# evanwang1990/FMwR

Measured on AMD Instinct MI355X. Metric: training examples/sec, 10Mx1M sparse FM SGD, higher is better.
Workload: dtype f32

## Files before the change

fmwr_amd/csrc/fm_batch_kernels.hip:

```cpp
#include <atomic>
#include <mutex>
#include <utility>
#include <vector>

#include "fmx_internal.h"
#include "fm_probit.h"
#include "fmx_test_hooks.h"

#ifndef FMX_U
#define FMX_U 4
#endif
#ifndef FMX_SPARSE_WAVES
#define FMX_SPARSE_WAVES 4
#endif
#ifndef FMX_DENSE_WAVES
#define FMX_DENSE_WAVES 4
#endif
#ifndef FMX_U_LARGE
#define FMX_U_LARGE 4
#endif
#ifndef FMX_U_SMALL
#define FMX_U_SMALL 8
#endif

// ... 451 lines not shown
#pragma unroll
    for (int i = 0; i < VEC; ++i) pair += 0.5 * (sm[s][i] * sm[s][i] - qm[s][i]);
#pragma unroll
    for (int off = LPR / 2; off > 0; off >>= 1) pair += __shfl_xor(pair, off);
    const double y_hat = lin[s] + pair;
    if constexpr (TRAIN) {
      double mult = 0.0;
      if (have) {
        mult = grad_mult(h, y_hat, a.y[a.r0 + row]);
        float4 srow = slice_make(sm[s], T());
        srow = embed_store<LPR>(srow, lig, (float)mult, a.embed);
        *reinterpret_cast<float4*>(reinterpret_cast<T*>(a.S) + (size_t)row * KP + lig * VEC) = srow;
        if (lig == 0) reinterpret_cast<T*>(a.amul)[row] = (T)mult;
      }
      if (lig == 0) red[s * NG + eg] = mult;
    } else {
      if (have && lig == 0 && a.yhat) a.yhat[row] = link_apply(h, y_hat, a.link, a.pn_y);
    }
  }
  if constexpr (TRAIN) {
    __syncthreads();
    if (tid % 64 == 0) {
      const int s = tid / 64;
      if (R0 + (int64_t)s * NG < a.nrows) {
        double g0 = 0.0, q0 = 0.0;
        for (int i = 0; i < NG; ++i) { const double m = red[s * NG + i]; g0 += m; q0 += m * m; }
        a.partials[2 * ((size_t)blockIdx.x * MERGE_SLOTS + s)] = g0;
        a.partials[2 * ((size_t)blockIdx.x * MERGE_SLOTS + s) + 1] = q0;
      }
    }
  }
}

template <bool UNIFORM, bool PIPE>
__global__ __launch_bounds__(WG_THREADS, 4) void fm_rows_sched_k(RowsArgs a, Hyper h) {
  using T = float;
  constexpr int LPR = 4, VEC = 4, KP = LPR * VEC;
  constexpr int NG = WG_THREADS / LPR;
  constexpr int PER = MERGE_STAGE / WG_THREADS;
  static_assert(MERGE_STAGE == SCHED_STAGE_STEPS * NG && MERGE_SLOTS == 4, "the stage holds SCHED_STAGE_STEPS steps of one word per lane group");
  static_assert(UNIFORM || !PIPE, "only the unrolled walk has a round to request together");
  __shared__ uint32_t stage[MERGE_STAGE];
  __shared__ double red[MERGE_RPW];

  const int tid = threadIdx.x;
  const int gid = tid / LPR;
  const int lig = tid % LPR;
  const int64_t R0 = (int64_t)blockIdx.x * MERGE_RPW;
  const uint32_t w_lo = a.sched_dir[blockIdx.x], w_hi = a.sched_dir[blockIdx.x + 1];
  const int cnt = (w_hi - w_lo < (uint32_t)MERGE_STAGE) ? (int)(w_hi - w_lo) : MERGE_STAGE;
  const int steps = UNIFORM ? (cnt / NG) & ~3 : cnt / NG;
  {
    uint32_t id[PER];
#pragma unroll
    for (int u = 0; u < PER; ++u) {
      const int i = tid + u * WG_THREADS;
      id[u] = i < cnt ? a.sched[(size_t)w_lo + i] : SCHED_BUBBLE;
    }
#pragma unroll
    for (int u = 0; u < PER; ++u) {
      const int i = tid + u * WG_THREADS;
      if (i < cnt) stage[i] = id[u];
    }
  }
  __syncthreads();

  const __amdgpu_buffer_rsrc_t v_rsrc = table_rsrc(a.V, a.sched_vbytes);
  const __amdgpu_buffer_rsrc_t w_rsrc = table_rsrc(a.w ? a.w : a.V, a.w ? a.sched_wbytes : a.sched_vbytes);
  const bool k1 = h.k1 != 0;
  const int vsh = RowStride<T, LPR>::v(a.vsh) + 2, wsh = RowStride<T, LPR>::w(a.wsh) + 2;
  const uint32_t lane_off = (uint32_t)(lig * VEC * sizeof(T));
  double sm[MERGE_SLOTS][VEC], qm[MERGE_SLOTS][VEC], lin[MERGE_SLOTS];
#pragma unroll
  for (int s = 0; s < MERGE_SLOTS; ++s) {
#pragma unroll
    for (int i = 0; i < VEC; ++i) { sm[s][i] = 0.0; qm[s][i] = 0.0; }
    lin[s] = h.k0 ? a.scal[SC_W0] : 0.0;
  }
  const uint32_t* __restrict__ mine = stage + gid;

  if constexpr (UNIFORM) {
    for (int t = 0; t < steps; t += MERGE_SLOTS) {
// ... 28 lines not shown
        for (int i = 0; i < VEC; ++i) { tmp[i] = tmp[i] * x; tsq[i] = tmp[i] * tmp[i]; }
        if (k1) lin[j] += wx;
#pragma unroll
        for (int i = 0; i < VEC; ++i) { sm[j][i] += tmp[i]; qm[j][i] += tsq[i]; }
      }
    }
  } else {
    for (int t = 0; t < steps; ++t) {
      const uint32_t wd = mine[t * NG];
      const bool live = wd != SCHED_BUBBLE;
      const uint32_t c = wd & SCHED_MAX_P;
      const int esl = live ? (int)(wd >> 30) : MERGE_SLOTS;
      const float4 vv = buf_row(v_rsrc, live ? (c << vsh) + lane_off : BUF_SKIP, T());
      const T wv = buf_elem(w_rsrc, live ? c << wsh : BUF_SKIP, T());
      const double x = 1.0;
      const double wx = (double)wv * x;
      double tmp[VEC], tsq[VEC];
      slice_get(vv, tmp);
#pragma unroll
      for (int i = 0; i < VEC; ++i) { tmp[i] = tmp[i] * x; tsq[i] = tmp[i] * tmp[i]; }
#pragma unroll
      for (int s = 0; s < MERGE_SLOTS; ++s) {
        if (esl == s) {
          if (k1) lin[s] += wx;
#pragma unroll
          for (int i = 0; i < VEC; ++i) { sm[s][i] += tmp[i]; qm[s][i] += tsq[i]; }
        }
      }
    }
  }

  int eg = tid / LPR;
  asm volatile("" : "+v"(eg));
#pragma unroll
  for (int s = 0; s < MERGE_SLOTS; ++s) {
    const int64_t row = R0 + s * NG + eg;
    const bool have = row < a.nrows;
    double pair = 0.0;
#pragma unroll
    for (int i = 0; i < VEC; ++i) pair += 0.5 * (sm[s][i] * sm[s][i] - qm[s][i]);
#pragma unroll
    for (int off = LPR / 2; off > 0; off >>= 1) pair += __shfl_xor(pair, off);
    const double y_hat = lin[s] + pair;
    double mult = 0.0;
    if (have) {
      mult = grad_mult(h, y_hat, a.y[a.r0 + row]);
      float4 srow = slice_make(sm[s], T());
      srow = embed_store<LPR>(srow, lig, (float)mult, a.embed);
      *reinterpret_cast<float4*>(reinterpret_cast<T*>(a.S) + (size_t)row * KP + lig * VEC) = srow;
      if (lig == 0) reinterpret_cast<T*>(a.amul)[row] = (T)mult;
    }
    if (lig == 0) red[s * NG + eg] = mult;
  }
  __syncthreads();
  if (tid % 64 == 0) {
    const int s = tid / 64;
    if (R0 + (int64_t)s * NG < a.nrows) {
      double g0 = 0.0, q0 = 0.0;
      for (int i = 0; i < NG; ++i) { const double m = red[s * NG + i]; g0 += m; q0 += m * m; }
      a.partials[2 * ((size_t)blockIdx.x * MERGE_SLOTS + s)] = g0;
      a.partials[2 * ((size_t)blockIdx.x * MERGE_SLOTS + s) + 1] = q0;
    }
  }
}

template <typename T, int LPR, bool TRAIN>
__global__ __launch_bounds__(WG_THREADS) void fm_rows_forward_dyn_k(RowsArgs a, Hyper h) {
  using vec_t = typename Slice<T>::vec;
  constexpr int VEC = Slice<T>::N;
  constexpr int KP = LPR * VEC;
  constexpr int GROUPS = WG_THREADS / LPR;
  constexpr int RPW = 4 * GROUPS;
  constexpr int RU = FMX_U_LARGE;
  constexpr int PER = (RU + LPR - 1) / LPR;
  __shared__ int next_row;
  __shared__ double red[TRAIN ? RPW : 1];
  const int tid = threadIdx.x;
  const int grp = tid / LPR, lig = tid % LPR;
  const int lane0 = (tid & 63) - lig;
  const int64_t R0 = (int64_t)blockIdx.x * RPW;
  const int rows_here = (int)((R0 + RPW < a.nrows ? R0 + RPW : a.nrows) - R0);
  if (tid == 0) next_row = GROUPS;
  if (TRAIN) for (int i = tid; i < RPW; i += WG_THREADS) red[i] = 0.0;
  __syncthreads();
  const T* __restrict__ Vt = reinterpret_cast<const T*>(a.V) + lig * VEC;
// ... 433 lines not shown
template <bool TRAIN, int U>
static int launch_rows_merged_u(fmx_engine* e, const RowsArgs& a, int mode, bool* ran) {
  const size_t v_bytes = ((size_t)e->p << a.vsh) * sizeof(float);
  if (mode != 2 && (a.nrows < rows_merged_fill<TRAIN, U>(e) || a.col_skew != 1 || v_bytes <= MERGE_MIN_TABLE)) return FMX_OK;
  bool fits = false;
  FMX_TRY(rows_merged_fits(e, a, &fits));
  if (!fits) { g_rows_merged[1]++; return FMX_OK; }
  const int64_t grid = (a.nrows + MERGE_RPW - 1) / MERGE_RPW;
  FMX_CHECK(grid < (1LL << 31), FMX_ERR_INVALID, "rows_forward: grid too large (%lld)", (long long)grid);
  hipLaunchKernelGGL((fm_rows_merged_k<float, 4, TRAIN, U>), dim3((unsigned)grid), dim3(WG_THREADS), 0, e->stream, a, e->hyper);
  FMX_HIP(hipGetLastError());
  g_rows_merged[0]++;
  *ran = true;
  return FMX_OK;
}

template <bool TRAIN>
static int launch_rows_merged(fmx_engine* e, const RowsArgs& a, bool fp64_tables, bool* ran) {
  *ran = false;
  const int mode = rows_merge_mode();
  if (mode == 0 || fp64_tables || e->kp32 != 16 || !a.unit || a.qout || a.no_w || a.wg_threads == 64 || a.sort_rows || a.flat == 1) return FMX_OK;
  if (TRAIN && e->cfg.task == FMX_TASK_RANKING) return FMX_OK;
  if (a.nrows <= 0 || a.max_row_len <= 0 || a.mat_uid == 0) return FMX_OK;
  switch (rows_merge_u()) {
    case 2: return launch_rows_merged_u<TRAIN, 2>(e, a, mode, ran);
    default: return launch_rows_merged_u<TRAIN, 1>(e, a, mode, ran);
  }
}

#ifndef FMX_ROWS_SCHED_DEFAULT
#define FMX_ROWS_SCHED_DEFAULT 1
#endif
#ifndef FMX_ROWS_SCHED_POLICY_DEFAULT
#define FMX_ROWS_SCHED_POLICY_DEFAULT SCHED_MERGE
#endif
#ifndef FMX_ROWS_SCHED_RHO_DEFAULT
#define FMX_ROWS_SCHED_RHO_DEFAULT 1024
#endif
static std::atomic<int64_t> g_rows_sched[3];
void debug_rows_sched_launches(int64_t out[3]) {
  for (int i = 0; i < 3; ++i) out[i] = g_rows_sched[i].load();
}
void rows_sched_count_build() { g_rows_sched[2]++; }
static int rows_sched_mode() {
  static const int v = [] { const char* s = getenv("FMX_ROWS_SCHED"); return s ? atoi(s) : (getenv("FMX_ROWS_MERGE") ? 0 : FMX_ROWS_SCHED_DEFAULT); }();
  return v;
}
static int rows_sched_policy() {
  static const int v = [] {
    const char* s = getenv("FMX_ROWS_SCHED_POLICY");
    if (!s) return (int)FMX_ROWS_SCHED_POLICY_DEFAULT;
    return s[0] == 'm' ? (int)SCHED_MERGE : s[0] == 'f' ? (int)SCHED_FRONT : s[0] == 'r' ? (int)SCHED_ROUND : (int)FMX_ROWS_SCHED_POLICY_DEFAULT;
  }();
  return v;
}
static int rows_sched_rho_q() {
  static const int v = [] {
    const char* s = getenv("FMX_ROWS_SCHED_RHO");
    if (!s) return (int)FMX_ROWS_SCHED_RHO_DEFAULT;
    const double r = atof(s);
    return r <= 0.0 ? 0 : r >= 1.0 ? 1024 : (int)(r * 1024.0 + 0.5);
  }();
  return v;
}
static int rows_sched_u() { static const int v = [] { const char* s = getenv("FMX_ROWS_SCHED_U"); return (s && atoi(s) == 4) ? 4 : 1; }(); return v; }

bool rows_sched_wanted(fmx_engine* e, const RowsArgs& a, int* policy, int* rho_q) {
  const int mode = rows_sched_mode();
  if (mode == 0 || mb_wide(e) || e->kp32 != 16 || !a.unit || a.qout || a.no_w || a.wg_threads == 64 || a.sort_rows || a.flat == 1) return false;
  if (e->cfg.task == FMX_TASK_RANKING || a.nrows <= 0 || a.max_row_len <= 0 || a.mat_uid == 0 || !a.w) return false;
  const uint64_t v_bytes = (uint64_t)e->p * (uint64_t)a.vs * sizeof(float), w_bytes = (uint64_t)e->p * (uint64_t)a.ws * sizeof(float);
  if (v_bytes >= BUF_SKIP || w_bytes >= BUF_SKIP || e->p > SCHED_MAX_P) return false;
  if (mode != 2 && (a.nrows < rows_merged_fill<true, 1>(e) || a.col_skew != 1 || v_bytes <= MERGE_MIN_TABLE)) return false;
  *policy = rows_sched_policy();
  *rho_q = *policy == SCHED_MERGE ? 0 : rows_sched_rho_q();
  return true;
}

static int launch_rows_sched(fmx_engine* e, const RowsArgs& a_in, bool* ran) {
  *ran = false;
  if (a_in.sched_state == 0) return FMX_OK;
  int policy = 0, rho_q = 0;
  if (!rows_sched_wanted(e, a_in, &policy, &rho_q)) return FMX_OK;
  if (a_in.sched_state != 1 || !a_in.sched || !a_in.sched_dir) { g_rows_sched[1]++; return FMX_OK; }
  RowsArgs a = a_in;
  a.sched_vbytes = (uint32_t)((uint64_t)e->p * (uint64_t)a.vs * sizeof(float));
  a.sched_wbytes = (uint32_t)((((uint64_t)e->p - 1) * (uint64_t)a.ws + 1) * sizeof(float));
  const int64_t grid = (a.nrows + MERGE_RPW - 1) / MERGE_RPW;
  FMX_CHECK(grid < (1LL << 31), FMX_ERR_INVALID, "rows_forward: grid too large (%lld)", (long long)grid);
  if (!a.sched_uniform) hipLaunchKernelGGL((fm_rows_sched_k<false, false>), dim3((unsigned)grid), dim3(WG_THREADS), 0, e->stream, a, e->hyper);
  else if (rows_sched_u() == 4) hipLaunchKernelGGL((fm_rows_sched_k<true, true>), dim3((unsigned)grid), dim3(WG_THREADS), 0, e->stream, a, e->hyper);
  else hipLaunchKernelGGL((fm_rows_sched_k<true, false>), dim3((unsigned)grid), dim3(WG_THREADS), 0, e->stream, a, e->hyper);
  FMX_HIP(hipGetLastError());
  g_rows_sched[0]++;
  *ran = true;
  return FMX_OK;
}

int launch_rows_forward(fmx_engine* e, const RowsArgs& a_in, bool train, bool fp64_tables) {
  RowsArgs a = a_in;
  FMX_CHECK(a.vs >= (fp64_tables ? e->kp64 : e->kp32) && a.ws >= 1 && (a.vs & (a.vs - 1)) == 0 && (a.ws & (a.ws - 1)) == 0, FMX_ERR_STATE,
            "rows_forward: table strides not set (%d, %d)", a.vs, a.ws);
  {
    const int kp = fp64_tables ? e->kp64 : e->kp32;
    FMX_CHECK((!fp64_tables && kp <= WIR_MAX_KP) || (a.vs == kp && a.ws == 1), FMX_ERR_STATE, "rows_forward: strides (%d, %d) on a table of compiled strides (%d, 1)",
              a.vs, a.ws, kp);
  }
  a.vsh = __builtin_ctz((unsigned)a.vs); a.wsh = __builtin_ctz((unsigned)a.ws);
  static const bool embed_ok = [] { const char* v = getenv("FMX_EMBED_MULT"); return !(v && v[0] == '0'); }();
  static const int force = [] { const char* v = getenv("FMX_ROWS_SERIAL"); return v ? atoi(v) : -1; }();
  RowsTune& tu = e->rows_tune;
  auto pick = [&](const RowsArgs& r, int* serial, int* trial) -> int {
    *trial = -1;
    *serial = 1;
    if (force >= 0) { *serial = force; return FMX_OK; }
    const bool timed = r.wg_threads != 64 && r.nrows >= RowsTune::MIN_ROWS;
    const int64_t key = r.unit ? 1 : 0;
    if (timed && key != tu.key) {
      if (tu.events && tu.launches > 0 && tu.decided < 0) FMX_HIP(hipStreamSynchronize(e->stream));
      tu.key = key; tu.decided = -1; tu.launches = 0;
    }
    if (tu.decided >= 0) { *serial = tu.decided; return FMX_OK; }
    if (!timed) return FMX_OK;
// ... 1271 lines not shown
```

fmwr_amd/csrc/fm_ingest.hip:

```cpp
#include <hip/hip_runtime.h>

#include <atomic>
#include <mutex>
#include <thread>
#include <type_traits>
#include <vector>
#include <cstring>

#include <rocprim/rocprim.hpp>

#include "fmx_internal.h"

namespace fmx {

static std::atomic<int> g_fail_next_plan_build{0};
void debug_fail_next_plan_build() { g_fail_next_plan_build.store(1); }

__device__ __forceinline__ uint32_t entry_row(const int64_t* __restrict__ row_ptr, int64_t r0, int64_t nrows, int64_t base, int64_t t, int fixed_len) {
  if (fixed_len > 0) return (uint32_t)((t - base) / fixed_len);
  int64_t lo = r0, hi = r0 + nrows;
  while (hi - lo > 1) {
    const int64_t mid = (lo + hi) >> 1;
    if (row_ptr[mid] <= t) lo = mid; else hi = mid;
  }
// ... 1057 lines not shown
  FMX_HIP(hipHostMalloc(&L.h_counts, (size_t)(nt > 0 ? nt : 1) * 4 * sizeof(uint32_t)));
  PlanWorkspace ws;
  FMX_TRY(ws.reserve(max_cnt, m->p, stream));
  L.plans.resize((size_t)nt);
  for (int64_t t = 0; t < nt; ++t) {
    fmx_matrix::TilePlan& pl = L.plans[(size_t)t];
    const int64_t base = h_ptr[(size_t)t], cnt = h_ptr[(size_t)t + 1] - base;
    FMX_TRY(plan_alloc(pl, m->p, cnt, cnt >= (int64_t)m->p));
    pl.r0 = tile_start[(size_t)t]; pl.nrows = tile_start[(size_t)t + 1] - pl.r0; pl.base = base; pl.cnt = cnt;
    FMX_TRY(plan_build(pl, ws, m->p, m->row_ptr, m->col, m->val, L.brow, L.bval, stream, m->unit_values, m->fixed_row_len, m->dense_prefix,
                       m->field_base.empty() ? nullptr : &m->field_base));
    FMX_HIP(hipMemcpyAsync(L.h_counts + 4 * t, pl.dcounts, 4 * sizeof(uint32_t), hipMemcpyDeviceToHost, stream));
  }
  FMX_HIP(hipStreamSynchronize(stream));
  int64_t max_seg = 0;
  for (int64_t t = 0; t < nt; ++t) {
    plan_set_counts(L.plans[(size_t)t], m->p, L.h_counts + 4 * t);
    if ((int64_t)L.plans[(size_t)t].n_seg > max_seg) max_seg = L.plans[(size_t)t].n_seg;
  }
  m->plans.swap(L.plans);
  m->brow = L.brow; L.brow = nullptr;
  m->bval = L.bval; L.bval = nullptr;
  m->step_first_tile.swap(step_first);
  m->batch_rows = batch_rows; m->tile_rows = tile_rows; m->n_batches = nb;
  m->max_long_seg = max_seg; m->max_tile_cnt = max_cnt;
  m->plan_generation++;
  return FMX_OK;
}

constexpr int SCHED_IDS = 9216;
static std::atomic<uint32_t> g_sched_id_limit{SCHED_MAX_P};
void debug_rows_sched_id_limit(uint32_t limit) { g_sched_id_limit.store(limit ? limit : SCHED_MAX_P); }

template <bool WRITE>
__global__ __launch_bounds__(WG_THREADS) void rows_sched_k(const int64_t* __restrict__ row_ptr, const uint32_t* __restrict__ col, int64_t r0, int64_t nrows, uint32_t p,
                                                           int policy, uint32_t rho_q, uint32_t* __restrict__ steps, const uint32_t* __restrict__ dir,
                                                           uint32_t* __restrict__ words) {
  constexpr int NG = 64, SLOTS = 4, RPW = NG * SLOTS;
  __shared__ uint32_t ids[SCHED_IDS];
  __shared__ uint32_t most[NG];
  const int tid = threadIdx.x;
  const int64_t R0 = (int64_t)blockIdx.x * RPW;
  const int64_t R1 = R0 + RPW < nrows ? R0 + RPW : nrows;
  const int64_t lo = row_ptr[r0 + R0], hi = row_ptr[r0 + R1];
  const bool fits_lds = hi - lo <= SCHED_IDS;
  const int cnt = fits_lds ? (int)(hi - lo) : 0;
  for (int i = tid; i < cnt; i += WG_THREADS) ids[i] = col[lo + i];
  int pos[SLOTS], end[SLOTS], left = 0;
  if (tid < NG) {
#pragma unroll
    for (int s = 0; s < SLOTS; ++s) {
      const int64_t row = R0 + s * NG + tid;
      const int64_t ra = row < nrows ? row : nrows, rb = row + 1 < nrows ? row + 1 : nrows;
      const int64_t ta = row_ptr[r0 + ra] - lo, tb = row_ptr[r0 + rb] - lo;
      pos[s] = (int)(ta < cnt ? ta : cnt);
      end[s] = (int)(tb < cnt ? tb : cnt);
      left += end[s] - pos[s];
    }
    most[tid] = (uint32_t)left;
  }
  __syncthreads();
  if (tid >= NG) return;
  uint32_t E = 0;
  for (int i = 0; i < NG; ++i) E = most[i] > E ? most[i] : E;
  const uint64_t R = rho_q ? ((uint64_t)E * 1024u + rho_q - 1) / rho_q : 0;
  uint32_t T = 0;
  uint32_t* out = nullptr;
  if constexpr (WRITE) {
    T = (dir[blockIdx.x + 1] - dir[blockIdx.x]) / NG;
    out = words + dir[blockIdx.x] + tid;
  }
  const uint32_t cap = WRITE ? T : (uint32_t)SCHED_STAGE_STEPS + 1;
  uint32_t t = 0;
  for (; left > 0 && t < cap; ++t) {
    const uint32_t front = (R == 0 || (uint64_t)t + 1 >= R) ? 0xFFFFFFFFu : (uint32_t)(((uint64_t)t + 1) * p / R);
    int sel = -1;
    uint32_t best = 0;
    if (policy == SCHED_ROUND) {
      const int s = (int)(t & 3u);
#pragma unroll
      for (int j = 0; j < SLOTS; ++j)
        if (j == s && pos[j] < end[j]) { sel = j; best = ids[pos[j]]; }
    } else {
#pragma unroll
      for (int j = 0; j < SLOTS; ++j)
        if (pos[j] < end[j]) {
          const uint32_t c = ids[pos[j]];
          if (sel < 0 || c < best) { sel = j; best = c; }
        }
    }
    const bool take = sel >= 0 && best <= front;
    if (take) {
#pragma unroll
      for (int j = 0; j < SLOTS; ++j)
        if (j == sel) pos[j] += 1;
      left -= 1;
    }
    if constexpr (WRITE) out[(size_t)t * NG] = take ? (best | ((uint32_t)sel << 30)) : SCHED_BUBBLE;
  }
  if constexpr (WRITE) {
    for (; t < T; ++t) out[(size_t)t * NG] = SCHED_BUBBLE;
  } else {
    uint32_t mine = (left > 0 || !fits_lds) ? (uint32_t)SCHED_STAGE_STEPS + 1 : t;
    if (policy == SCHED_ROUND && mine <= (uint32_t)SCHED_STAGE_STEPS) mine = (mine + 3u) & ~3u;
    atomicMax(&steps[blockIdx.x], mine);
  }
}

void rows_sched_free(fmx_matrix* m) {
  (void)hipFree(m->rows_sched.words);
  (void)hipFree(m->rows_sched.dir);
  m->rows_sched = fmx_matrix::RowsSched{};
}

int rows_sched_build(fmx_matrix* m, int policy, int rho_q, hipStream_t stream) {
  auto& S = m->rows_sched;
  if (S.tried && S.generation == m->plan_generation && S.policy == policy && S.rho_q == rho_q) return FMX_OK;
  rows_sched_free(m);
  S.tried = 1; S.generation = m->plan_generation; S.policy = policy; S.rho_q = rho_q;
  const size_t nt = m->plans.size();
  S.tile_words.assign(nt, -1);
  S.tile_dir.assign(nt, 0);
  if (m->refilled_in_place || nt == 0 || m->p > g_sched_id_limit.load() || !m->unit_values) return FMX_OK;
  FMX_CHECK(policy >= SCHED_MERGE && policy <= SCHED_ROUND && rho_q >= 0 && rho_q <= 1024, FMX_ERR_INVALID, "rows_sched_build: policy %d, rho %d/1024", policy, rho_q);
  if (policy == SCHED_MERGE) rho_q = 0;
  FMX_HIP(hipSetDevice(m->device));
  timespec t0, t1;
  clock_gettime(CLOCK_MONOTONIC, &t0);
  int64_t slots = 0;
  for (size_t t = 0; t < nt; ++t) { S.tile_dir[t] = slots; slots += (m->plans[t].nrows + 255) / 256 + 1; }
  uint32_t* d_dir = nullptr;
  FMX_HIP(hipMalloc(&d_dir, (size_t)slots * sizeof(uint32_t)));
  S.dir = d_dir;
  FMX_HIP(hipMemsetAsync(d_dir, 0, (size_t)slots * sizeof(uint32_t), stream));
  for (size_t t = 0; t < nt; ++t) {
    const auto& pl = m->plans[t];
    const int64_t blocks = (pl.nrows + 255) / 256;
    if (blocks <= 0) continue;
    FMX_CHECK(blocks < (1LL << 31), FMX_ERR_INVALID, "rows_sched_build: %lld blocks in a tile", (long long)blocks);
    hipLaunchKernelGGL((rows_sched_k<false>), dim3((unsigned)blocks), dim3(WG_THREADS), 0, stream, m->row_ptr, m->col, pl.r0, pl.nrows, m->p, policy, (uint32_t)rho_q,
                       d_dir + S.tile_dir[t] + 1, (const uint32_t*)nullptr, (uint32_t*)nullptr);
  }
  FMX_HIP(hipGetLastError());
  std::vector<uint32_t> h((size_t)slots);
  FMX_HIP(hipMemcpyAsync(h.data(), d_dir, (size_t)slots * sizeof(uint32_t), hipMemcpyDeviceToHost, stream));
  FMX_HIP(hipStreamSynchronize(stream));
  int64_t total = 0;
  for (size_t t = 0; t < nt; ++t) {
    const int64_t blocks = (m->plans[t].nrows + 255) / 256;
    uint32_t* d = h.data() + S.tile_dir[t];
    bool fits = blocks > 0;
    for (int64_t b = 1; b <= blocks; ++b) fits = fits && d[b] <= (uint32_t)SCHED_STAGE_STEPS;
    if (!fits) continue;
    uint32_t at = 0;
    for (int64_t b = 1; b <= blocks; ++b) { const uint32_t steps = d[b]; d[b - 1] = at; at += steps * 64u; }
    d[blocks] = at;
    S.tile_words[t] = total;
    total += at;
  }
  bool any = false;
  for (const int64_t v : S.tile_words) any = any || v >= 0;
  if (!any) return FMX_OK;
  FMX_HIP(hipMemcpyAsync(d_dir, h.data(), (size_t)slots * sizeof(uint32_t), hipMemcpyHostToDevice, stream));
  if (hipMalloc(&S.words, (size_t)(total > 0 ? total : 1) * sizeof(uint32_t)) != hipSuccess) {
    (void)hipGetLastError();
    FMX_HIP(hipStreamSynchronize(stream));
    (void)hipFree(S.dir);
    S.words = nullptr; S.dir = nullptr;
    S.tile_words.assign(nt, -1);
    return FMX_OK;
  }
  S.bytes = (size_t)(total > 0 ? total : 1) * sizeof(uint32_t) + (size_t)slots * sizeof(uint32_t);
  for (size_t t = 0; t < nt; ++t) {
    if (S.tile_words[t] < 0) continue;
    const auto& pl = m->plans[t];
    const int64_t blocks = (pl.nrows + 255) / 256;
    hipLaunchKernelGGL((rows_sched_k<true>), dim3((unsigned)blocks), dim3(WG_THREADS), 0, stream, m->row_ptr, m->col, pl.r0, pl.nrows, m->p, policy, (uint32_t)rho_q,
                       (uint32_t*)nullptr, (const uint32_t*)(d_dir + S.tile_dir[t]), S.words + S.tile_words[t]);
  }
  FMX_HIP(hipGetLastError());
  FMX_HIP(hipStreamSynchronize(stream));
  clock_gettime(CLOCK_MONOTONIC, &t1);
  S.build_ms = 1e3 * (double)(t1.tv_sec - t0.tv_sec) + 1e-6 * (double)(t1.tv_nsec - t0.tv_nsec);
  rows_sched_count_build();
  return FMX_OK;
}

int debug_rows_sched_export(const fmx_matrix* m, int64_t tile, int64_t block, uint32_t* out, int64_t cap_words, int64_t* steps) {
  const auto& S = m->rows_sched;
  FMX_CHECK(steps != nullptr, FMX_ERR_INVALID, "steps is NULL");
  *steps = -1;
  if (!S.words || S.generation != m->plan_generation || tile < 0 || tile >= (int64_t)S.tile_words.size() || S.tile_words[(size_t)tile] < 0) return FMX_OK;
  const int64_t blocks = (m->plans[(size_t)tile].nrows + 255) / 256;
  FMX_CHECK(block >= 0 && block < blocks, FMX_ERR_INVALID, "block %lld out of range (0..%lld)", (long long)block, (long long)blocks - 1);
  FMX_HIP(hipSetDevice(m->device));
  uint32_t d[2];
  FMX_HIP(hipMemcpy(d, S.dir + S.tile_dir[(size_t)tile] + block, sizeof(d), hipMemcpyDeviceToHost));
  const int64_t n = (int64_t)d[1] - (int64_t)d[0];
  *steps = n / 64;
  FMX_CHECK(out != nullptr && n <= cap_words, FMX_ERR_INVALID, "the block's %lld words do not fit %lld", (long long)n, (long long)cap_words);
  if (n > 0) FMX_HIP(hipMemcpy(out, S.words + S.tile_words[(size_t)tile] + d[0], (size_t)n * sizeof(uint32_t), hipMemcpyDeviceToHost));
  return FMX_OK;
}

struct MergeWs {
  int64_t cap = 0;
  int n_parts_cap = 0;
  uint32_t *keys_in = nullptr, *keys_out = nullptr, *pos_in = nullptr, *pos_out = nullptr, *roff = nullptr, *rfeat = nullptr, *dcount = nullptr;
  uint32_t* blk = nullptr;
  void* sort_temp = nullptr; size_t sort_bytes = 0;
};

void merge_ws_free(MergeWs* w) {
  if (!w) return;
  (void)hipFree(w->keys_in); (void)hipFree(w->keys_out); (void)hipFree(w->pos_in); (void)hipFree(w->pos_out); (void)hipFree(w->roff);
  (void)hipFree(w->rfeat); (void)hipFree(w->dcount); (void)hipFree(w->blk); (void)hipFree(w->sort_temp);
  delete w;
}

static int merge_ws_reserve(fmx_engine* e, int64_t total, int n_parts) {
  if (!e->merge) e->merge = new MergeWs();
  MergeWs& w = *e->merge;
  if (total <= w.cap && n_parts <= w.n_parts_cap) return FMX_OK;
  FMX_HIP(hipStreamSynchronize(e->stream));
  MergeWs* old = e->merge;
  e->merge = new MergeWs();
  merge_ws_free(old);
  MergeWs& n = *e->merge;
  const size_t m = (size_t)(total > 0 ? total : 1) * 5 / 4 + 64;
  FMX_HIP(hipMalloc(&n.keys_in, m * 4)); FMX_HIP(hipMalloc(&n.keys_out, m * 4));
  FMX_HIP(hipMalloc(&n.pos_in, m * 4)); FMX_HIP(hipMalloc(&n.pos_out, m * 4));
  FMX_HIP(hipMalloc(&n.roff, (m + 1) * 4)); FMX_HIP(hipMalloc(&n.rfeat, m * 4));
// ... 993 lines not shown
```

fmwr_amd/csrc/fmx_api.hip:

```cpp
#include <algorithm>
#include <cmath>
#include <cstdlib>
#include <cstring>
#include <ctime>
#include <atomic>
#include <memory>

#include "fmx_internal.h"
#include "fmx_test_hooks.h"
#include "fm_probit.h"

namespace fmx {

static thread_local std::string g_error;

void set_error(const char* fmt, ...) {
  char buf[1024];
  va_list ap;
  va_start(ap, fmt);
  vsnprintf(buf, sizeof(buf), fmt, ap);
  va_end(ap);
  g_error = buf;
}

// ... 294 lines not shown
    left -= nrows;
    total += nrows;
  }
  *step_rows = total;
  return FMX_OK;
}

static int rows_phase(fmx_engine* e, fmx_matrix* m, const TileRun& t, int64_t step_rows, int64_t partial_offset, int64_t* n_partials, int64_t s_row0 = 0) {
  RowsArgs a{};
  a.row_ptr = m->row_ptr; a.col = m->col; a.val = m->val; a.y = m->y;
  a.r0 = t.r0; a.nrows = t.nrows;
  a.V = mb_vbase(e); a.w = mb_wbase(e); a.vs = mb_vstride(e); a.ws = mb_wstride(e);
  a.scal = e->scal;
  a.S = (char*)e->S + (size_t)s_row0 * mb_kp(e) * mb_elem(e);
  a.amul = (char*)e->amul + (size_t)s_row0 * mb_elem(e);
  a.partials = e->partials + 2 * partial_offset;
  a.unit = m->unit_values;
  a.sort_rows = rows_ragged(m);
  a.wg_threads = rows_wg_threads(step_rows, mb_lpr(e));
  a.split = rows_split(step_rows, mb_lpr(e));
  a.flat = rows_flat(m); a.nmat = m->n;
  a.mat_uid = m->uid; a.max_row_len = m->max_row_len; a.col_skew = rows_col_skew(m, m->plans[(size_t)t.tile]);
  {
    int policy = 0, rho_q = 0;
    if (rows_sched_wanted(e, a, &policy, &rho_q)) {
      FMX_TRY(rows_sched_build(m, policy, rho_q, e->stream));
      const auto& S = m->rows_sched;
      const auto& pl = m->plans[(size_t)t.tile];
      if (S.dir && S.generation == m->plan_generation && (size_t)t.tile < S.tile_words.size() && pl.r0 == t.r0 && pl.nrows == t.nrows) {
        if (S.tile_words[(size_t)t.tile] >= 0) {
          a.sched = S.words + S.tile_words[(size_t)t.tile];
          a.sched_dir = S.dir + S.tile_dir[(size_t)t.tile];
          a.sched_uniform = S.policy == SCHED_ROUND ? 1 : 0;
          a.sched_state = 1;
        } else a.sched_state = 2;
      }
    }
  }
  const int rpw = a.wg_threads / (mb_lpr(e) * (a.wg_threads == 64 && a.split == 4 ? 4 : 1));
  *n_partials = (a.flat == 1 && !a.sort_rows && a.wg_threads != 64) ? rows_flat_blocks(t.r0, t.nrows, rpw) : (t.nrows + rpw - 1) / rpw;
  return launch_rows_forward(e, a, true, mb_wide(e));
}

static int cols_args(fmx_engine* e, fmx_matrix* m, const TileRun& t, bool sparse_ok, ColsArgs* out) {
  const auto& pl = m->plans[(size_t)t.tile];
  ColsArgs c{};
  c.brow = m->brow + pl.base;
  c.bval = m->bval + pl.base;
  c.rows_active = (uint32_t)t.nrows;
  c.walk = 1;
  c.unit = m->unit_values;
  if (pl.feat && sparse_ok) {
    c.tfeat = pl.feat; c.toff = pl.soff; c.n_tfeat = pl.n_lists;
    c.trow0 = pl.row0; c.tval0 = pl.val0;
    c.list_entries = pl.cnt;
  } else {
    if (!pl.off) FMX_TRY(plan_ensure_dense(m, t.tile, e->stream));
    c.bptr = m->plans[(size_t)t.tile].off;
    c.list_entries = m->plans[(size_t)t.tile].cnt;
  }
  *out = c;
  return FMX_OK;
}

static int long_args(fmx_engine* e, fmx_matrix* m, int64_t tile, LongArgs* la, ColsArgs* c) {
  const auto& pl = m->plans[(size_t)tile];
// ... 1701 lines not shown
```

fmwr_amd/csrc/fmx_internal.h:

```cpp
#pragma once
#include <hip/hip_runtime.h>

#include <cstdarg>
#include <cstdint>
#include <cstdio>
#include <cstdlib>
#include <functional>
#include <string>
#include <utility>
#include <vector>

#include "../../include/fmx.h"

namespace fmx {

void set_error(const char* fmt, ...);

#define FMX_HIP(call)                                                                         \
  do {                                                                                        \
    hipError_t _e = (call);                                                                   \
    if (_e != hipSuccess) {                                                                   \
      fmx::set_error("%s failed: %s (%s:%d)", #call, hipGetErrorString(_e), __FILE__, __LINE__); \
      return FMX_ERR_HIP;                                                                     \
    }                                                                                         \
// ... 296 lines not shown
  const float* y;
  int64_t r0;
  int64_t nrows;
  const void* V;
  const void* w;
  int vs, ws;
  int vsh, wsh;
  const double* scal;
  void* S;
  void* amul;
  double* partials;
  double* yhat;
  double* qout;
  int64_t qout_t;
  const double* pn_y;
  int link;
  int unit;
  int no_w;
  int embed;
  int wg_threads;
  int split;
  int serial;
  int flat;
  int64_t nmat;
  int sort_rows;
  uint64_t mat_uid;
  int max_row_len;
  int col_skew;
  const uint32_t* sched;
  const uint32_t* sched_dir;
  int sched_state;
  uint32_t sched_vbytes, sched_wbytes;
  int sched_uniform;
  int fixed_schedule;
};
constexpr size_t FMX_SERIAL_TABLE_MAX = 1ull << 30;
inline int rows_wg_threads(int64_t step_rows, int lpr) { return step_rows * lpr < 512LL * WG_THREADS ? 64 : WG_THREADS; }
inline int rows_split(int64_t step_rows, int lpr) { return (lpr <= 16 && step_rows * lpr < 1024LL * 64) ? 4 : 1; }
inline int rows_ragged(const fmx_matrix* m) {
  const char* s = getenv("FMX_ROWS_PULL");
  return (s && s[0] == '1' && m->fixed_row_len == 0 && m->n > 0) ? 1 : 0;
}
inline int rows_flat(const fmx_matrix* m) {
  if (m->fixed_row_len != 0 || m->n <= 0 || m->nnz <= 0) return 0;
  if ((int64_t)m->max_row_len * WG_THREADS >= (1LL << 31)) return 0;
  const char* s = getenv("FMX_ROWS_FLAT");
  return (s && s[0] == '1') ? 1 : 0;
}
inline int64_t rows_flat_blocks(int64_t r0, int64_t nrows, int g) { return nrows > 0 ? (r0 + nrows - 1) / g - r0 / g + 1 : 0; }
inline int rows_col_skew(const fmx_matrix* m, const fmx_matrix::TilePlan& pl) {
  const uint64_t lists = pl.feat ? pl.n_lists : m->p;
  if (lists == 0 || pl.n_long == 0) return 1;
  return ((uint64_t)pl.cnt <= 32ull * lists && (uint64_t)pl.n_long * 1024ull >= lists) ? 2 : 1;
}
int launch_rows_forward(fmx_engine* e, const RowsArgs& a, bool train, bool fp64_tables);
enum RowsSchedPolicy : int { SCHED_MERGE = 0, SCHED_FRONT = 1, SCHED_ROUND = 2 };
constexpr int SCHED_STAGE_STEPS = 144;
constexpr uint32_t SCHED_BUBBLE = 0xFFFFFFFFu;
constexpr uint32_t SCHED_MAX_P = (1u << 30) - 1;
bool rows_sched_wanted(fmx_engine* e, const RowsArgs& a, int* policy, int* rho_q);
void rows_sched_count_build();
void debug_rows_sched_launches(int64_t out[3]);
int rows_sched_build(fmx_matrix* m, int policy, int rho_q, hipStream_t stream);
void rows_sched_free(fmx_matrix* m);
void debug_rows_sched_id_limit(uint32_t limit);
int debug_rows_sched_export(const fmx_matrix* m, int64_t tile, int64_t block, uint32_t* out, int64_t cap_words, int64_t* steps);
int ensure_probit(fmx_engine* e);
int topk_run(fmx_engine* e, const fmx_matrix* C, int64_t r0, int64_t r1, const fmx_matrix* I, const fmx_matrix* X, int K, int link, int64_t* d_index,
             double* d_score);
int heldout_run(fmx_engine* e, const fmx_matrix* C, int64_t r0, int64_t r1, const fmx_matrix* I, const fmx_matrix* H, const fmx_matrix* X, int64_t* d_rank,
                double* d_score, const int32_t* ks, int n_ks, double* pc);
int heldout_means(fmx_engine* e, const double* pc, int64_t n, int cols, double* out, int64_t* counted);
void debug_heldout_limits(int window, int64_t chunk);
int lists_run(fmx_engine* e, const fmx_matrix* C, int64_t r0, int64_t r1, const fmx_matrix* I, const fmx_matrix* Lm, int link, int K, double* d_score,
              int64_t* d_pos, int64_t* d_index, double* d_tscore);
int project_run(fmx_engine* e, const fmx_matrix* m, int64_t r0, int64_t r1, bool with_w0, double* d_base, double* d_s);
void debug_lists_limits(int lds_entries, int64_t chunk);
int diversify_run(fmx_engine* e, const fmx_matrix* I, int64_t n, int P, const int64_t* index, const double* score, int K, double lambda, int relevance,
                  int64_t* oi, double* os, double* om, bool host);
void debug_diversify_limits(int lds_rows, int64_t chunk);
int neighbors_run(fmx_engine* e, const fmx_matrix* Q, int64_t r0, int64_t r1, const fmx_matrix* I, int K, int metric, bool skip_self, int64_t* d_index,
                  double* d_score);
void debug_neighbors_limits(int64_t slice_items, int64_t chunk_rows);
int contrib_run(fmx_engine* e, const fmx_matrix* m, int64_t r0, int64_t r1, double* d_out);
int pairs_build(const fmx_matrix* C, const fmx_matrix* I, const fmx_matrix* X, int n_neg, uint64_t seed, int64_t epoch, fmx_matrix** out,
                fmx_engine* e = nullptr, int n_cand = 1);
void debug_pairs_hard_chunk(int64_t contexts);
int contrib_summary_run(fmx_engine* e, const fmx_matrix* m, double* sum, double* abs_sum, int64_t* count);
int foldin_run(fmx_engine* e, const fmx_matrix* m, const uint32_t* ids, int64_t n_ids, double lw, double lv, int n_newton, bool pairs,
// ... 248 lines not shown
```

Before: 1.035 billion.

## Add DEAL schedule policy that assigns rows to lane-group slots to balance column sweeps

Adds a new SCHED_DEAL policy and makes it the default. The schedule builder bins each row's feature ids into 16 cuts and greedily deals rows to lane-group slots so the merged column streams follow an even ramp across the table. A per-block header of row placements is stored ahead of the schedule words, and the train kernel reads it to map slots to rows. The aim is to keep concurrent waves touching nearby V/w cache lines and so cut table refetches. In exchange it adds schedule-build work, one extra header word per lane group, and an indirection when writing outputs.

```diff
diff --git a/fmwr_amd/csrc/fm_batch_kernels.hip b/fmwr_amd/csrc/fm_batch_kernels.hip
--- a/fmwr_amd/csrc/fm_batch_kernels.hip
+++ b/fmwr_amd/csrc/fm_batch_kernels.hip
@@ -507,7 +507,7 @@
   }
 }
 
-template <bool UNIFORM, bool PIPE>
+template <bool UNIFORM, bool PIPE, bool DEAL = false>
 __global__ __launch_bounds__(WG_THREADS, 4) void fm_rows_sched_k(RowsArgs a, Hyper h) {
   using T = float;
   constexpr int LPR = 4, VEC = 4, KP = LPR * VEC;
@@ -515,14 +515,22 @@
   constexpr int PER = MERGE_STAGE / WG_THREADS;
   static_assert(MERGE_STAGE == SCHED_STAGE_STEPS * NG && MERGE_SLOTS == 4, "the stage holds SCHED_STAGE_STEPS steps of one word per lane group");
   static_assert(UNIFORM || !PIPE, "only the unrolled walk has a round to request together");
+  static_assert(!(UNIFORM && DEAL), "a DEAL schedule is walked as a MERGE one");
   __shared__ uint32_t stage[MERGE_STAGE];
   __shared__ double red[MERGE_RPW];
+  __shared__ uint32_t places[DEAL ? NG : 1];
 
   const int tid = threadIdx.x;
   const int gid = tid / LPR;
   const int lig = tid % LPR;
   const int64_t R0 = (int64_t)blockIdx.x * MERGE_RPW;
-  const uint32_t w_lo = a.sched_dir[blockIdx.x], w_hi = a.sched_dir[blockIdx.x + 1];
+  const uint32_t w_hi = a.sched_dir[blockIdx.x + 1];
+  uint32_t w_lo = a.sched_dir[blockIdx.x];
+  if constexpr (DEAL) {
+    const bool hdr = w_hi - w_lo >= (uint32_t)NG;
+    if (tid < NG) places[tid] = hdr ? a.sched[(size_t)w_lo + tid] : 0u;
+    w_lo += hdr ? (uint32_t)NG : 0u;
+  }
   const int cnt = (w_hi - w_lo < (uint32_t)MERGE_STAGE) ? (int)(w_hi - w_lo) : MERGE_STAGE;
   const int steps = UNIFORM ? (cnt / NG) & ~3 : cnt / NG;
   {
@@ -617,9 +625,12 @@
 
   int eg = tid / LPR;
   asm volatile("" : "+v"(eg));
+  uint32_t place = 0;
+  if constexpr (DEAL) place = places[eg];
 #pragma unroll
   for (int s = 0; s < MERGE_SLOTS; ++s) {
-    const int64_t row = R0 + s * NG + eg;
+    const int at = DEAL ? (int)((place >> (8 * s)) & 255u) : s * NG + eg;
+    const int64_t row = R0 + at;
     const bool have = row < a.nrows;
     double pair = 0.0;
 #pragma unroll
@@ -635,7 +646,7 @@
       *reinterpret_cast<float4*>(reinterpret_cast<T*>(a.S) + (size_t)row * KP + lig * VEC) = srow;
       if (lig == 0) reinterpret_cast<T*>(a.amul)[row] = (T)mult;
     }
-    if (lig == 0) red[s * NG + eg] = mult;
+    if (lig == 0) red[at] = mult;
   }
   __syncthreads();
   if (tid % 64 == 0) {
@@ -1135,7 +1146,7 @@
 #define FMX_ROWS_SCHED_DEFAULT 1
 #endif
 #ifndef FMX_ROWS_SCHED_POLICY_DEFAULT
-#define FMX_ROWS_SCHED_POLICY_DEFAULT SCHED_MERGE
+#define FMX_ROWS_SCHED_POLICY_DEFAULT SCHED_DEAL
 #endif
 #ifndef FMX_ROWS_SCHED_RHO_DEFAULT
 #define FMX_ROWS_SCHED_RHO_DEFAULT 1024
@@ -1153,7 +1164,7 @@
   static const int v = [] {
     const char* s = getenv("FMX_ROWS_SCHED_POLICY");
     if (!s) return (int)FMX_ROWS_SCHED_POLICY_DEFAULT;
-    return s[0] == 'm' ? (int)SCHED_MERGE : s[0] == 'f' ? (int)SCHED_FRONT : s[0] == 'r' ? (int)SCHED_ROUND : (int)FMX_ROWS_SCHED_POLICY_DEFAULT;
+    return s[0] == 'm' ? (int)SCHED_MERGE : s[0] == 'f' ? (int)SCHED_FRONT : s[0] == 'r' ? (int)SCHED_ROUND : s[0] == 'd' ? (int)SCHED_DEAL : (int)FMX_ROWS_SCHED_POLICY_DEFAULT;
   }();
   return v;
 }
@@ -1176,7 +1187,7 @@
   if (v_bytes >= BUF_SKIP || w_bytes >= BUF_SKIP || e->p > SCHED_MAX_P) return false;
   if (mode != 2 && (a.nrows < rows_merged_fill<true, 1>(e) || a.col_skew != 1 || v_bytes <= MERGE_MIN_TABLE)) return false;
   *policy = rows_sched_policy();
-  *rho_q = *policy == SCHED_MERGE ? 0 : rows_sched_rho_q();
+  *rho_q = (*policy == SCHED_MERGE || *policy == SCHED_DEAL) ? 0 : rows_sched_rho_q();
   return true;
 }
 
@@ -1191,7 +1202,8 @@
   a.sched_wbytes = (uint32_t)((((uint64_t)e->p - 1) * (uint64_t)a.ws + 1) * sizeof(float));
   const int64_t grid = (a.nrows + MERGE_RPW - 1) / MERGE_RPW;
   FMX_CHECK(grid < (1LL << 31), FMX_ERR_INVALID, "rows_forward: grid too large (%lld)", (long long)grid);
-  if (!a.sched_uniform) hipLaunchKernelGGL((fm_rows_sched_k<false, false>), dim3((unsigned)grid), dim3(WG_THREADS), 0, e->stream, a, e->hyper);
+  if (a.sched_deal) hipLaunchKernelGGL((fm_rows_sched_k<false, false, true>), dim3((unsigned)grid), dim3(WG_THREADS), 0, e->stream, a, e->hyper);
+  else if (!a.sched_uniform) hipLaunchKernelGGL((fm_rows_sched_k<false, false>), dim3((unsigned)grid), dim3(WG_THREADS), 0, e->stream, a, e->hyper);
   else if (rows_sched_u() == 4) hipLaunchKernelGGL((fm_rows_sched_k<true, true>), dim3((unsigned)grid), dim3(WG_THREADS), 0, e->stream, a, e->hyper);
   else hipLaunchKernelGGL((fm_rows_sched_k<true, false>), dim3((unsigned)grid), dim3(WG_THREADS), 0, e->stream, a, e->hyper);
   FMX_HIP(hipGetLastError());
diff --git a/fmwr_amd/csrc/fm_ingest.hip b/fmwr_amd/csrc/fm_ingest.hip
--- a/fmwr_amd/csrc/fm_ingest.hip
+++ b/fmwr_amd/csrc/fm_ingest.hip
@@ -1113,7 +1113,10 @@
 static std::atomic<uint32_t> g_sched_id_limit{SCHED_MAX_P};
 void debug_rows_sched_id_limit(uint32_t limit) { g_sched_id_limit.store(limit ? limit : SCHED_MAX_P); }
 
-template <bool WRITE>
+constexpr int DEAL_CUTS = 16;
+static_assert(((int64_t)4096 * SCHED_IDS + (int64_t)4 * DEAL_CUTS * SCHED_IDS) < (1LL << 26), "a pick's cost << 6 | lane group fits 32 bits for a block within the stage");
+
+template <bool WRITE, bool DEAL>
 __global__ __launch_bounds__(WG_THREADS) void rows_sched_k(const int64_t* __restrict__ row_ptr, const uint32_t* __restrict__ col, int64_t r0, int64_t nrows, uint32_t p,
                                                            int policy, uint32_t rho_q, uint32_t* __restrict__ steps, const uint32_t* __restrict__ dir,
                                                            uint32_t* __restrict__ words) {
@@ -1141,6 +1144,91 @@
     most[tid] = (uint32_t)left;
   }
   __syncthreads();
+  uint32_t hdr = 0;
+  if constexpr (DEAL) {
+    __shared__ int32_t exc[RPW * DEAL_CUTS];
+    __shared__ uint32_t key[RPW];
+    __shared__ uint8_t order[RPW];
+    {
+      const int64_t row = R0 + tid;
+      const int64_t ra = row < nrows ? row : nrows, rb = row + 1 < nrows ? row + 1 : nrows;
+      const int64_t ta = row_ptr[r0 + ra] - lo, tb = row_ptr[r0 + rb] - lo;
+      const int e0 = (int)(ta < cnt ? ta : cnt), e1 = (int)(tb < cnt ? tb : cnt);
+      uint32_t q[DEAL_CUTS - 1];
+      int32_t c[DEAL_CUTS];
+#pragma unroll
+      for (int k = 1; k < DEAL_CUTS; ++k) { q[k - 1] = (uint32_t)(((uint64_t)k * p) >> 4); c[k - 1] = 0; }
+      c[DEAL_CUTS - 1] = e1 - e0;
+      for (int e = e0; e < e1; ++e) {
+        const uint32_t v = ids[e];
+#pragma unroll
+        for (int k = 0; k < DEAL_CUTS - 1; ++k) c[k] += v < q[k] ? 1 : 0;
+      }
+      uint32_t kmax = 0;
+#pragma unroll
+      for (int k = 0; k < DEAL_CUTS; ++k) {
+        const int32_t a = 4096 * c[k] - (k + 1) * cnt;
+        exc[tid * DEAL_CUTS + k] = a;
+        const uint32_t m = (uint32_t)(a < 0 ? -a : a);
+        kmax = m > kmax ? m : kmax;
+      }
+      key[tid] = kmax;
+    }
+    __syncthreads();
+    {
+      const uint32_t mine = key[tid];
+      int rank = 0;
+      for (int j = 0; j < RPW; ++j) {
+        const uint32_t o = key[j];
+        rank += (o > mine || (o == mine && j < tid)) ? 1 : 0;
+      }
+      order[rank] = (uint8_t)tid;
+    }
+    __syncthreads();
+    if (tid >= NG) return;
+    int32_t A[DEAL_CUTS];
+#pragma unroll
+    for (int k = 0; k < DEAL_CUTS; ++k) A[k] = 0;
+    for (int level = 0; level < SLOTS; ++level) {
+      bool taken = false;
+      for (int j = 0; j < NG; ++j) {
+        const int i = order[level * NG + j];
+        int32_t a[DEAL_CUTS];
+#pragma unroll
+        for (int k = 0; k < DEAL_CUTS; ++k) a[k] = exc[i * DEAL_CUTS + k];
+        uint32_t cost = 0;
+#pragma unroll
+        for (int k = 0; k < DEAL_CUTS; ++k) {
+          const int32_t v = A[k] + a[k];
+          const uint32_t m = (uint32_t)(v < 0 ? -v : v);
+          cost = m > cost ? m : cost;
+        }
+        const uint32_t bid = taken ? 0xFFFFFFFFu : ((cost << 6) | (uint32_t)tid);
+        uint32_t best = bid;
+#pragma unroll
+        for (int off = 32; off > 0; off >>= 1) {
+          const uint32_t o = (uint32_t)__shfl_xor((int)best, off);
+          best = o < best ? o : best;
+        }
+        if (best == bid) {
+          taken = true;
+          hdr |= (uint32_t)i << (8 * level);
+#pragma unroll
+          for (int k = 0; k < DEAL_CUTS; ++k) A[k] += a[k];
+        }
+      }
+    }
+    left = 0;
+#pragma unroll
+    for (int s = 0; s < SLOTS; ++s) {
+      const int64_t row = R0 + (int64_t)((hdr >> (8 * s)) & 255u);
+      const int64_t ra = row < nrows ? row : nrows, rb = row + 1 < nrows ? row + 1 : nrows;
+      const int64_t ta = row_ptr[r0 + ra] - lo, tb = row_ptr[r0 + rb] - lo;
+      pos[s] = (int)(ta < cnt ? ta : cnt);
+      end[s] = (int)(tb < cnt ? tb : cnt);
+      left += end[s] - pos[s];
+    }
+  }
   if (tid >= NG) return;
   uint32_t E = 0;
   for (int i = 0; i < NG; ++i) E = most[i] > E ? most[i] : E;
@@ -1150,6 +1238,7 @@
   if constexpr (WRITE) {
     T = (dir[blockIdx.x + 1] - dir[blockIdx.x]) / NG;
     out = words + dir[blockIdx.x] + tid;
+    if constexpr (DEAL) { *out = hdr; out += NG; T -= 1; }
   }
   const uint32_t cap = WRITE ? T : (uint32_t)SCHED_STAGE_STEPS + 1;
   uint32_t t = 0;
@@ -1203,8 +1292,10 @@
   S.tile_words.assign(nt, -1);
   S.tile_dir.assign(nt, 0);
   if (m->refilled_in_place || nt == 0 || m->p > g_sched_id_limit.load() || !m->unit_values) return FMX_OK;
-  FMX_CHECK(policy >= SCHED_MERGE && policy <= SCHED_ROUND && rho_q >= 0 && rho_q <= 1024, FMX_ERR_INVALID, "rows_sched_build: policy %d, rho %d/1024", policy, rho_q);
-  if (policy == SCHED_MERGE) rho_q = 0;
+  FMX_CHECK(policy >= SCHED_MERGE && policy <= SCHED_DEAL && rho_q >= 0 && rho_q <= 1024, FMX_ERR_INVALID, "rows_sched_build: policy %d, rho %d/1024", policy, rho_q);
+  if (policy == SCHED_MERGE || policy == SCHED_DEAL) rho_q = 0;
+  const bool deal = policy == SCHED_DEAL;
+  const uint32_t hdr_words = deal ? 64u : 0u;
   FMX_HIP(hipSetDevice(m->device));
   timespec t0, t1;
   clock_gettime(CLOCK_MONOTONIC, &t0);
@@ -1219,8 +1310,10 @@
     const int64_t blocks = (pl.nrows + 255) / 256;
     if (blocks <= 0) continue;
     FMX_CHECK(blocks < (1LL << 31), FMX_ERR_INVALID, "rows_sched_build: %lld blocks in a tile", (long long)blocks);
-    hipLaunchKernelGGL((rows_sched_k<false>), dim3((unsigned)blocks), dim3(WG_THREADS), 0, stream, m->row_ptr, m->col, pl.r0, pl.nrows, m->p, policy, (uint32_t)rho_q,
-                       d_dir + S.tile_dir[t] + 1, (const uint32_t*)nullptr, (uint32_t*)nullptr);
+    if (deal) hipLaunchKernelGGL((rows_sched_k<false, true>), dim3((unsigned)blocks), dim3(WG_THREADS), 0, stream, m->row_ptr, m->col, pl.r0, pl.nrows, m->p, policy, (uint32_t)rho_q,
+                                 d_dir + S.tile_dir[t] + 1, (const uint32_t*)nullptr, (uint32_t*)nullptr);
+    else hipLaunchKernelGGL((rows_sched_k<false, false>), dim3((unsigned)blocks), dim3(WG_THREADS), 0, stream, m->row_ptr, m->col, pl.r0, pl.nrows, m->p, policy, (uint32_t)rho_q,
+                            d_dir + S.tile_dir[t] + 1, (const uint32_t*)nullptr, (uint32_t*)nullptr);
   }
   FMX_HIP(hipGetLastError());
   std::vector<uint32_t> h((size_t)slots);
@@ -1234,7 +1327,7 @@
     for (int64_t b = 1; b <= blocks; ++b) fits = fits && d[b] <= (uint32_t)SCHED_STAGE_STEPS;
     if (!fits) continue;
     uint32_t at = 0;
-    for (int64_t b = 1; b <= blocks; ++b) { const uint32_t steps = d[b]; d[b - 1] = at; at += steps * 64u; }
+    for (int64_t b = 1; b <= blocks; ++b) { const uint32_t steps = d[b]; d[b - 1] = at; at += hdr_words + steps * 64u; }
     d[blocks] = at;
     S.tile_words[t] = total;
     total += at;
@@ -1256,8 +1349,10 @@
     if (S.tile_words[t] < 0) continue;
     const auto& pl = m->plans[t];
     const int64_t blocks = (pl.nrows + 255) / 256;
-    hipLaunchKernelGGL((rows_sched_k<true>), dim3((unsigned)blocks), dim3(WG_THREADS), 0, stream, m->row_ptr, m->col, pl.r0, pl.nrows, m->p, policy, (uint32_t)rho_q,
-                       (uint32_t*)nullptr, (const uint32_t*)(d_dir + S.tile_dir[t]), S.words + S.tile_words[t]);
+    if (deal) hipLaunchKernelGGL((rows_sched_k<true, true>), dim3((unsigned)blocks), dim3(WG_THREADS), 0, stream, m->row_ptr, m->col, pl.r0, pl.nrows, m->p, policy, (uint32_t)rho_q,
+                                 (uint32_t*)nullptr, (const uint32_t*)(d_dir + S.tile_dir[t]), S.words + S.tile_words[t]);
+    else hipLaunchKernelGGL((rows_sched_k<true, false>), dim3((unsigned)blocks), dim3(WG_THREADS), 0, stream, m->row_ptr, m->col, pl.r0, pl.nrows, m->p, policy, (uint32_t)rho_q,
+                            (uint32_t*)nullptr, (const uint32_t*)(d_dir + S.tile_dir[t]), S.words + S.tile_words[t]);
   }
   FMX_HIP(hipGetLastError());
   FMX_HIP(hipStreamSynchronize(stream));
@@ -1278,7 +1373,7 @@
   uint32_t d[2];
   FMX_HIP(hipMemcpy(d, S.dir + S.tile_dir[(size_t)tile] + block, sizeof(d), hipMemcpyDeviceToHost));
   const int64_t n = (int64_t)d[1] - (int64_t)d[0];
-  *steps = n / 64;
+  *steps = n / 64 - (S.policy == SCHED_DEAL ? 1 : 0);
   FMX_CHECK(out != nullptr && n <= cap_words, FMX_ERR_INVALID, "the block's %lld words do not fit %lld", (long long)n, (long long)cap_words);
   if (n > 0) FMX_HIP(hipMemcpy(out, S.words + S.tile_words[(size_t)tile] + d[0], (size_t)n * sizeof(uint32_t), hipMemcpyDeviceToHost));
   return FMX_OK;
diff --git a/fmwr_amd/csrc/fmx_api.hip b/fmwr_amd/csrc/fmx_api.hip
--- a/fmwr_amd/csrc/fmx_api.hip
+++ b/fmwr_amd/csrc/fmx_api.hip
@@ -350,6 +350,7 @@
           a.sched = S.words + S.tile_words[(size_t)t.tile];
           a.sched_dir = S.dir + S.tile_dir[(size_t)t.tile];
           a.sched_uniform = S.policy == SCHED_ROUND ? 1 : 0;
+          a.sched_deal = S.policy == SCHED_DEAL ? 1 : 0;
           a.sched_state = 1;
         } else a.sched_state = 2;
       }
diff --git a/fmwr_amd/csrc/fmx_internal.h b/fmwr_amd/csrc/fmx_internal.h
--- a/fmwr_amd/csrc/fmx_internal.h
+++ b/fmwr_amd/csrc/fmx_internal.h
@@ -352,6 +352,7 @@
   int sched_state;
   uint32_t sched_vbytes, sched_wbytes;
   int sched_uniform;
+  int sched_deal;
   int fixed_schedule;
 };
 constexpr size_t FMX_SERIAL_TABLE_MAX = 1ull << 30;
@@ -374,7 +375,7 @@
   return ((uint64_t)pl.cnt <= 32ull * lists && (uint64_t)pl.n_long * 1024ull >= lists) ? 2 : 1;
 }
 int launch_rows_forward(fmx_engine* e, const RowsArgs& a, bool train, bool fp64_tables);
-enum RowsSchedPolicy : int { SCHED_MERGE = 0, SCHED_FRONT = 1, SCHED_ROUND = 2 };
+enum RowsSchedPolicy : int { SCHED_MERGE = 0, SCHED_FRONT = 1, SCHED_ROUND = 2, SCHED_DEAL = 3 };
 constexpr int SCHED_STAGE_STEPS = 144;
 constexpr uint32_t SCHED_BUBBLE = 0xFFFFFFFFu;
 constexpr uint32_t SCHED_MAX_P = (1u << 30) - 1;
diff --git a/profiles/rows_deal_sim.py b/profiles/rows_deal_sim.py
--- /dev/null
+++ b/profiles/rows_deal_sim.py
@@ -0,0 +1,84 @@
+import argparse
+import os
+import sys
+import time
+
+import numpy as np
+
+sys.path.insert(0, os.path.dirname(os.path.dirname(os.path.abspath(__file__))))
+from tests import rows_deal_model as D
+
+P, NNZ, BLOCKS, NG, SLOTS, LRU_LINES, XCDS = 1_000_000, 30, 128, 64, 4, 32768, 8
+W_BASE = 1 << 40
+
+
+def streams(rng, kind):
+    if kind == "even":
+        n = SLOTS * NNZ
+        band = np.arange(n, dtype=np.float64) * P / n
+        return (band[None, :] + rng.random((BLOCKS * NG, n)) * P / n).astype(np.int64)
+    out = np.empty((BLOCKS * NG, SLOTS * NNZ), np.int64)
+    for b in range(BLOCKS):
+        rows = np.sort(rng.integers(0, P, (256, NNZ)), axis=1)
+        if kind == "deal":
+            m = D.deal_map([[int(c) for c in r] for r in rows], P)
+        else:
+            m = D.identity_map()
+        for g in range(NG):
+            out[b * NG + g] = np.sort(np.concatenate([rows[m[s][g]] for s in range(SLOTS)]))
+    return out
+
+
+def excursion(cols):
+    n = cols.shape[1]
+    ramp = (np.arange(n) + 0.5) * P / n
+    return float(np.mean(np.max(np.abs(cols - ramp[None, :]), axis=1)) / P)
+
+
+def lines_fetched(cols, drift, rng):
+    n_streams, n = cols.shape
+    offset = np.repeat(rng.normal(0.0, drift, n_streams // 16) if drift > 0 else np.zeros(n_streams // 16), 16)
+    when = (np.arange(n, dtype=np.float64)[None, :] + offset[:, None]).ravel()
+    order = np.argsort(when, kind="stable")
+    flat = cols.ravel()[order]
+    v_line, w_line = (flat >> 1).tolist(), ((flat >> 5) + W_BASE).tolist()
+    lru, miss_v, miss_w = {}, 0, 0
+    for v, w in zip(v_line, w_line):
+        for key in (v, w):
+            if key in lru:
+                del lru[key]
+            else:
+                if key >= W_BASE:
+                    miss_w += 1
+                else:
+                    miss_v += 1
+                if len(lru) >= LRU_LINES:
+                    del lru[next(iter(lru))]
+            lru[key] = None
+    return miss_v, miss_w
+
+
+def main():
+    ap = argparse.ArgumentParser()
+    ap.add_argument("--drift", type=float, nargs="*", default=[0.0, 2.0, 4.0, 8.0], help="sd of a wave's offset against the common clock, in steps")
+    ap.add_argument("--seed", type=int, default=1)
+    a = ap.parse_args()
+    t0 = time.time()
+    sets = {}
+    for kind in ("identity", "deal", "even"):
+        sets[kind] = streams(np.random.default_rng(a.seed), kind)
+    print(f"streams made in {time.time() - t0:.1f} s; mean largest excursion from the ramp, fraction of p: " + ", ".join(f"{k} {excursion(v):.4f}" for k, v in sets.items()))
+    distinct = len(np.unique(sets["identity"] >> 1))
+    print(f"distinct V lines one XCD touches: {distinct} ({XCDS * distinct / 1e6:.2f} M per tile: perfect re-use)")
+    print("M lines per tile (8 XCDs):   drift   identity V / w      DEAL V / w      even V / w")
+    for d in a.drift:
+        row = []
+        for kind in ("identity", "deal", "even"):
+            v, w = lines_fetched(sets[kind], d, np.random.default_rng(a.seed + 1000))
+            row.append(f"{XCDS * v / 1e6:6.2f} / {XCDS * w / 1e6:4.2f}")
+        print(f"                             {d:5.1f}   " + "   ".join(row), flush=True)
+    print(f"{time.time() - t0:.1f} s")
+
+
+if __name__ == "__main__":
+    main()
```

Result: faster. 1.070 billion (median of 6 runs) (+3.4%).
